# xuanvinh1997/llm-fp8

Hardware: AMD Instinct MI355X
Metric: train tokens/sec + FP8 GEMM % of MFMA peak, Llama-3.2-3B seq512 b16 (higher is better)
Workload: dtype fp8 (E4M3/E5M2 operands, fp32 accumulate, bf16 activations); 1 GPU; llama-3.2-3b (28 layers) full fine-tuning step, batch 16/GPU x seq 512, fp8_scenario=default (te_llama counterpart, lm_head FP8 under the outer recipe), random-init weights, synthetic tokens; route=fused, global_batch=16, seq_len=512, parallelism=single

## Files before the change

include/mi_fp8.h:

```cpp
#ifndef MI_FP8_H
#define MI_FP8_H

#include <stdint.h>

#ifdef __cplusplus
extern "C" {
#endif

#define MI_FMT_E4M3 0
#define MI_FMT_E5M2 1

#define MI_OK 0
#define MI_ERR_ARG (-1)
#define MI_ERR_SHAPE (-2)
#define MI_ERR_HIP (-3)

#define MI_OUT_BF16 0
#define MI_OUT_F32 1

#define MI_AMAX_ALGO_MAX 0
#define MI_AMAX_ALGO_MOST_RECENT 1

#define MI_ABI_VERSION 5
int mi_abi_version(void);
// ... 97 lines not shown
                        void* yT_fp8, const float* scale, float* amax, int64_t rows, int64_t cols, int fmt, void* stream);

int mi_sumsq_bf16(const void* g_bf16, int64_t n, float* partial, int n_partials, void* stream);
int mi_sumsq_bf16_multi(const int64_t* table, int n_tensors, const int32_t* chunks, int n_chunks, int chunk_elems,
                        double* partial, void* stream);
int mi_adamw_bf16_multi(const int64_t* table, int n_tensors, const int32_t* chunks, int n_chunks, int chunk_elems,
                        const float* grad_scale, float lr, float beta1, float beta2, float eps, float weight_decay,
                        int64_t step, void* stream);
int mi_adamw_cast_bf16_multi(const int64_t* table, int n_tensors, const int32_t* chunks, int n_chunks, int chunk_elems,
                             const float* grad_scale, float lr, float beta1, float beta2, float eps, float weight_decay,
                             int64_t step, void* stream);
int mi_adamw_mxcast_bf16_multi(const int64_t* table, int n_tensors, const int32_t* chunks, int n_chunks, int chunk_elems,
                               const float* grad_scale, float lr, float beta1, float beta2, float eps, float weight_decay,
                               int64_t step, void* stream);

int mi_embedding_grad_add(void* grad_bf16, const void* dy_bf16, const int64_t* sorted_ids, const int64_t* perm, int64_t tokens,
                          int64_t hidden, int64_t vocab, float alpha, int64_t padding_idx, void* stream);
int mi_adamw_bf16(void* p_bf16, const void* g_bf16, void* exp_avg_bf16, void* exp_avg_sq_bf16, int64_t n,
                  const float* grad_scale, float lr, float beta1, float beta2, float eps, float weight_decay,
                  int64_t step, void* stream);

int mi_attn_fwd(const void* q, const void* k, const void* v, void* o, float* lse, int B, int S, int H, int G, int D,
                int64_t q_ts, int64_t k_ts, int64_t v_ts, int64_t o_ts, float scale, int causal, void* stream);
#ifdef MI_DIAG
int mi_attn_fwd_diag(const void* q, const void* k, const void* v, void* o, float* lse, unsigned long long* dbg, int B, int S,
                     int H, int G, int D, int64_t q_ts, int64_t k_ts, int64_t v_ts, int64_t o_ts, float scale, void* stream);
#endif
int mi_attn_bwd(const void* q, const void* k, const void* v, const void* o, const void* dout, const float* lse,
                float* delta, void* dq, void* dk, void* dv, int B, int S, int H, int G, int D, int64_t q_ts,
                int64_t k_ts, int64_t v_ts, int64_t o_ts, int64_t do_ts, int64_t dq_ts, int64_t dk_ts, int64_t dv_ts,
                float scale, int causal, void* stream);

#ifdef __cplusplus
}
#endif
#endif
```

llm_fp8_amd/_lib.py:

```python
from __future__ import annotations

import ctypes
import os

_HERE = os.path.dirname(os.path.abspath(__file__))
LIB_PATH = os.environ.get("LLM_FP8_AMD_LIB") or os.path.join(_HERE, "libmi_fp8.so")
LAB_LIB_PATH = os.path.join(os.path.dirname(_HERE), "tools", "bin", "libmi_fp8_lab.so")

MI_FMT_E4M3 = 0
MI_FMT_E5M2 = 1
ABI_VERSION = 5

_c_i64 = ctypes.c_int64
_c_int = ctypes.c_int
_p = ctypes.c_void_p

class GemmProblem(ctypes.Structure):
    _fields_ = [("A", ctypes.c_void_p), ("B", ctypes.c_void_p), ("D", ctypes.c_void_p), ("sa_inv", ctypes.c_void_p),
                ("sb_inv", ctypes.c_void_p), ("M", ctypes.c_int64), ("N", ctypes.c_int64), ("K", ctypes.c_int64),
                ("lda", ctypes.c_int64), ("ldb", ctypes.c_int64), ("ldd", ctypes.c_int64)]


class GemmMxProblem(ctypes.Structure):
    _fields_ = [("A", ctypes.c_void_p), ("SA", ctypes.c_void_p), ("B", ctypes.c_void_p), ("SB", ctypes.c_void_p),
# ... 22 lines not shown
    "mi_rmsnorm_bwd": [_p, _p, _p, _p, _p, _p, _p, _c_int, _c_i64, _c_i64, _p],
    "mi_ce_forward": [_p, _p, _p, _p, _c_i64, _c_i64, _p],
    "mi_ce_backward": [_p, _p, _p, _p, _p, _c_i64, _c_i64, _p],
    "mi_ce_backward_cast": [_p, _p, _p, _p, _p, _p, _p, _p, _c_i64, _c_i64, _c_int, _p],
    "mi_sumsq_bf16": [_p, _c_i64, _p, _c_int, _p],
    "mi_sumsq_bf16_multi": [_p, _c_int, _p, _c_int, _c_int, _p, _p],
    "mi_adamw_bf16_multi": [_p, _c_int, _p, _c_int, _c_int, _p, ctypes.c_float, ctypes.c_float, ctypes.c_float, ctypes.c_float,
                            ctypes.c_float, _c_i64, _p],
    "mi_adamw_cast_bf16_multi": [_p, _c_int, _p, _c_int, _c_int, _p, ctypes.c_float, ctypes.c_float, ctypes.c_float, ctypes.c_float,
                                 ctypes.c_float, _c_i64, _p],
    "mi_adamw_mxcast_bf16_multi": [_p, _c_int, _p, _c_int, _c_int, _p, ctypes.c_float, ctypes.c_float, ctypes.c_float, ctypes.c_float,
                                   ctypes.c_float, _c_i64, _p],
    "mi_embedding_grad_add": [_p, _p, _p, _p, _c_i64, _c_i64, _c_i64, ctypes.c_float, _c_i64, _p],
    "mi_adamw_bf16": [_p, _p, _p, _p, _c_i64, _p, ctypes.c_float, ctypes.c_float, ctypes.c_float, ctypes.c_float,
                      ctypes.c_float, _c_i64, _p],
    "mi_add_rmsnorm_stats": [_p, _p, _p, _p, _c_i64, _c_i64, ctypes.c_float, _p],
    "mi_cast_amax_colsum": [_p, _p, _p, _p, _p, _p, _c_i64, _c_i64, _c_i64, _c_i64, _c_int, _p],
    "mi_colsum_finish": [_p, _c_i64, _c_i64, _p, _c_int, _p],
    "mi_colsum_finish_multi": [_p, _p, _p, _p, _p, _c_int, _p],
    "mi_gemm_workspace_bytes": [],
    "mi_gemm_set_workspace": [_p, _c_i64],
    "mi_attn_fwd": [_p, _p, _p, _p, _p, _c_int, _c_int, _c_int, _c_int, _c_int, _c_i64, _c_i64, _c_i64, _c_i64, ctypes.c_float,
                    _c_int, _p],
    "mi_attn_bwd": [_p] * 10 + [_c_int] * 5 + [_c_i64] * 8 + [ctypes.c_float, _c_int, _p],
    "mi_mxfp8_norm_quantize": [_p, _p, _p, _p, _p, _p, _p, _c_i64, _c_i64, _c_int, _p],
    "mi_mxfp8_swiglu_quantize": [_p, _p, _p, _p, _p, _c_i64, _c_i64, _c_int, _p],
    "mi_mxfp8_dswiglu_quantize": [_p, _p, _p, _p, _p, _p, _p, _c_i64, _c_i64, _c_int, _p],
    "mi_gemm_mxfp8": [_p, _p, _p, _p, _p, _p, _c_i64, _c_i64, _c_i64, _c_int, _c_int, _c_int, _c_int, _p],
    "mi_swiglu_cast_bias": [_p, _p, _p, _p, _p, _p, _c_i64, _c_i64, _c_int, _p],
    "mi_dswiglu_cast_bias": [_p, _p, _p, _p, _p, _p, _p, _p, _c_i64, _c_i64, _c_int, _p],
    "mi_add_bias_rmsnorm_stats": [_p, _p, _p, _p, _p, _c_i64, _c_i64, ctypes.c_float, _p],
    "mi_gemm_fp8_clock": [_p, _p, _p, _p, _p, _c_i64, _c_i64, _c_i64, _c_i64, _c_i64, _c_i64, _c_int, _p, _p],
}
LAB_SIGNATURES = {
    "mi_attn_fwd_diag": [_p, _p, _p, _p, _p, _p, _c_int, _c_int, _c_int, _c_int, _c_int, _c_i64, _c_i64, _c_i64, _c_i64, ctypes.c_float, _p],
}

_lib = None


def _bind(path: str, signatures) -> ctypes.CDLL:
    lib = ctypes.CDLL(path)
    for name, argtypes in signatures.items():
        fn = getattr(lib, name)
        fn.argtypes = argtypes
        fn.restype = ctypes.c_char_p if name == "mi_last_error" else (_c_i64 if name == "mi_gemm_workspace_bytes" else _c_int)
# ... 37 lines not shown
```

llm_fp8_amd/csrc/mi_attn.hip:

```cpp
#include "mi_common.h"

namespace mi {

typedef __bf16 bf8 __attribute__((ext_vector_type(8)));
typedef short s4v __attribute__((ext_vector_type(4)));
typedef short s8v __attribute__((ext_vector_type(8)));
typedef float f16v __attribute__((ext_vector_type(16)));
typedef __attribute__((address_space(3))) s4v lds_s4v;

template <int D>
__device__ __forceinline__ int tile_off(int row, int ch) {
  if (D == 128) return 256 * row + 16 * (ch ^ (((row & 3) << 2) | ((row >> 2) & 3)));
  return 128 * row + 16 * (ch ^ (((row & 1) << 2) | ((row >> 1) & 3)));
}

__device__ __forceinline__ bf8 as_bf8(v4i v) { return __builtin_bit_cast(bf8, v); }

template <int D>
__device__ __forceinline__ bf8 row_frag(const char* tile, int r0, int t, int lane) {
  const int r = lane & 31, h = lane >> 5;
  return as_bf8(*reinterpret_cast<const v4i*>(tile + tile_off<D>(r0 + r, 2 * t + h)));
}

template <int D>
// ... 28 lines not shown
constexpr int ATT_KB = 64;

typedef __amdgpu_buffer_rsrc_t rsrc_t;
#define MI_LDS_PTR(p) ((__attribute__((address_space(3))) void*)(p))
template <int D>
__device__ __forceinline__ void dma_voffsets(int* voff, int64_t tok_stride, int tid) {
  const int lane = tid & 63, w = tid >> 6;
#pragma unroll
  for (int i = 0; i < D / 32; ++i) {
    const int p = (4 * i + w) * 1024 + 16 * lane;
    const int row = p / (2 * D), slot = (p % (2 * D)) / 16;
    const int ch = D == 128 ? slot ^ (((row & 3) << 2) | ((row >> 2) & 3)) : slot ^ (((row & 1) << 2) | ((row >> 1) & 3));
    voff[i] = (int)((int64_t)row * tok_stride * 2) + 16 * ch;
  }
}
template <int D>
__device__ __forceinline__ void stage_dma(rsrc_t rs, const int* voff, int soff, char* tile, int w) {
#pragma unroll
  for (int i = 0; i < D / 32; ++i)
    __builtin_amdgcn_raw_ptr_buffer_load_lds(rs, MI_LDS_PTR(tile + (4 * i + w) * 1024), 16, voff[i], soff, 0, 0);
}
__device__ __forceinline__ void dma_wait_all() { asm volatile("s_waitcnt vmcnt(0)" ::: "memory"); }

template <int D, bool CAUSAL, bool DIAG = false>
__global__ __launch_bounds__(256, 2) void attn_fwd_kernel(const uint16_t* __restrict__ q, const uint16_t* __restrict__ k,
                                                          const uint16_t* __restrict__ v, uint16_t* __restrict__ o,
                                                          float* __restrict__ lse, int S, int H, int G, int64_t q_ts,
                                                          int64_t k_ts, int64_t v_ts, int64_t o_ts, float c,
                                                          unsigned long long* __restrict__ dbg = nullptr) {
  constexpr int TILE = ATT_KB * D * 2;
  constexpr int KT = D / 16, DB = D / 32;
  __shared__ __attribute__((aligned(16))) char lds[4 * TILE];
  const int tid = threadIdx.x, lane = tid & 63, w = tid >> 6, r = lane & 31, h = lane >> 5;
  const int qb = gridDim.x - 1 - blockIdx.x, head = blockIdx.y, b = blockIdx.z, g = head / (H / G);
  const int q_first = qb * ATT_QB + w * 32;
  const int qrow = q_first + r;
  const int ntiles = CAUSAL ? (qb * ATT_QB + ATT_QB) / ATT_KB : S / ATT_KB;
  const uint16_t* kbase = k + (int64_t)b * S * k_ts + (int64_t)g * D;
  const uint16_t* vbase = v + (int64_t)b * S * v_ts + (int64_t)g * D;

  bf8 qf[KT];
  {
    const uint16_t* qp = q + ((int64_t)b * S + qrow) * q_ts + (int64_t)head * D + 8 * h;
#pragma unroll
    for (int t = 0; t < KT; ++t) qf[t] = as_bf8(*reinterpret_cast<const v4i*>(qp + 16 * t));
  }
#pragma unroll
  for (int t = 0; t < KT; ++t) retire(qf[t]);
  f16v oacc[DB];
#pragma unroll
  for (int d = 0; d < DB; ++d)
#pragma unroll
// ... 119 lines not shown

  l += __shfl_xor(l, 32);
  const float inv = 1.0f / l;
  if (h == 0) lse[((int64_t)b * H + head) * S + qrow] = m * c + __builtin_amdgcn_logf(l);
  char* ot = lds + w * (32 * D * 2);
#pragma unroll
  for (int d = 0; d < DB; ++d)
#pragma unroll
    for (int i = 0; i < 4; ++i) {
      const int ch = 4 * d + i;
      uint2 pk;
      pk.x = pack_bf16x2(oacc[d][4 * i] * inv, oacc[d][4 * i + 1] * inv);
      pk.y = pack_bf16x2(oacc[d][4 * i + 2] * inv, oacc[d][4 * i + 3] * inv);
      *reinterpret_cast<uint2*>(ot + r * (D * 2) + 16 * (ch ^ (r & (D / 8 - 1))) + 8 * h) = pk;
    }
  __builtin_amdgcn_s_waitcnt(0xc07f);
  __builtin_amdgcn_wave_barrier();
  constexpr int CPR = D / 8;
#pragma unroll
  for (int it = 0; it < 32 * CPR / 64; ++it) {
    const int idx = it * 64 + lane, row = idx / CPR, ch = idx % CPR;
    const v4i val = *reinterpret_cast<const v4i*>(ot + row * (D * 2) + 16 * (ch ^ (row & (CPR - 1))));
    *reinterpret_cast<v4i*>(o + ((int64_t)b * S + q_first + row) * o_ts + (int64_t)head * D + ch * 8) = val;
  }
}


template <int D>
__device__ __forceinline__ void store_rows_from_accT(const f16v (&acc)[D / 32], float mul, char* slice, uint16_t* out,
                                                     int64_t row_stride, int lane) {
  const int r = lane & 31, h = lane >> 5;
  constexpr int CPR = D / 8;
#pragma unroll
  for (int d = 0; d < D / 32; ++d)
#pragma unroll
    for (int i = 0; i < 4; ++i) {
      const int ch = 4 * d + i;
      uint2 pk;
      pk.x = pack_bf16x2(acc[d][4 * i] * mul, acc[d][4 * i + 1] * mul);
      pk.y = pack_bf16x2(acc[d][4 * i + 2] * mul, acc[d][4 * i + 3] * mul);
      *reinterpret_cast<uint2*>(slice + r * (D * 2) + 16 * (ch ^ (r & (CPR - 1))) + 8 * h) = pk;
    }
  __builtin_amdgcn_s_waitcnt(0xc07f);
  __builtin_amdgcn_wave_barrier();
#pragma unroll
  for (int it = 0; it < 32 * CPR / 64; ++it) {
// ... 240 lines not shown
        const bf8 pf = acc_frag(sacc, s), dsf = acc_frag(dsacc, s);
#pragma unroll
        for (int d = 0; d < DB; ++d) {
          dva[d] = __builtin_amdgcn_mfma_f32_32x32x16_bf16(tr_frag<D>(dt, 16 * s, 32 * d, lane), pf, dva[d], 0, 0, 0);
          dka[d] = __builtin_amdgcn_mfma_f32_32x32x16_bf16(tr_frag<D>(qt, 16 * s, 32 * d, lane), dsf, dka[d], 0, 0, 0);
        }
      }
    }
    if (D == 128) {
#pragma unroll
      for (int d = 0; d < DB; ++d) asm volatile("" : "+a"(dka[d]), "+a"(dva[d]));
    }
    if (more) store_step(lds + ((step + 1) & 1) * BUF);
    __syncthreads();
  }
  char* slice = lds + w * SL;
  store_rows_from_accT<D>(dka, scale, slice, dk + ((int64_t)b * S + key_first) * dk_ts + (int64_t)g * D, dk_ts, lane);
  __builtin_amdgcn_wave_barrier();
  store_rows_from_accT<D>(dva, 1.0f, slice, dv + ((int64_t)b * S + key_first) * dv_ts + (int64_t)g * D, dv_ts, lane);
}

}

extern "C" int mi_attn_fwd(const void* q, const void* k, const void* v, void* o, float* lse, int B, int S, int H, int G,
                           int D, int64_t q_ts, int64_t k_ts, int64_t v_ts, int64_t o_ts, float scale, int causal,
                           void* stream) {
  MI_CHECK_ARG(q && k && v && o && lse, "mi_attn_fwd: null pointer");
  MI_CHECK_ARG(B >= 1 && H >= 1 && G >= 1 && H % G == 0, "mi_attn_fwd: bad B/H/G (%d, %d, %d)", B, H, G);
  MI_CHECK_ARG(D == 128 || D == 64, "mi_attn_fwd: head_dim %d not supported (64, 128)", D);
  MI_CHECK_ARG(S >= 128 && S % 128 == 0, "mi_attn_fwd: seq %d must be a multiple of 128", S);
  MI_CHECK_ARG(q_ts % 8 == 0 && k_ts % 8 == 0 && v_ts % 8 == 0 && o_ts % 8 == 0, "mi_attn_fwd: token strides must be multiples of 8");
  MI_CHECK_ARG((int64_t)S * k_ts * 2 < (1LL << 31) && (int64_t)S * v_ts * 2 < (1LL << 31) && ((uintptr_t)k % 16) == 0 && ((uintptr_t)v % 16) == 0,
               "mi_attn_fwd: one batch of K / V must span < 2 GiB and be 16-byte aligned (32-bit buffer offsets of the LDS DMA)");
  MI_CHECK_ARG(((uintptr_t)q % 16) == 0 && ((uintptr_t)o % 16) == 0, "mi_attn_fwd: q and o must be 16-byte aligned (16-byte row accesses)");
  MI_CHECK_ARG(H <= 65535 && B <= 65535, "mi_attn_fwd: grid too large");
  const float c = scale * 1.4426950408889634f;
  dim3 grid(S / mi::ATT_QB, H, B), block(256);
  hipStream_t st = (hipStream_t)stream;
#define MI_ATTN_FWD(DD, CC)                                                                                            \
  hipLaunchKernelGGL((mi::attn_fwd_kernel<DD, CC>), grid, block, 0, st, (const uint16_t*)q, (const uint16_t*)k,          \
                     (const uint16_t*)v, (uint16_t*)o, lse, S, H, G, q_ts, k_ts, v_ts, o_ts, c, (unsigned long long*)nullptr)
  if (D == 128) {
    if (causal) MI_ATTN_FWD(128, true); else MI_ATTN_FWD(128, false);
  } else {
    if (causal) MI_ATTN_FWD(64, true); else MI_ATTN_FWD(64, false);
  }
#undef MI_ATTN_FWD
  MI_CHECK_LAUNCH("mi_attn_fwd launch");
  return MI_OK;
}

#ifdef MI_DIAG
extern "C" int mi_attn_fwd_diag(const void* q, const void* k, const void* v, void* o, float* lse, unsigned long long* dbg, int B,
                                int S, int H, int G, int D, int64_t q_ts, int64_t k_ts, int64_t v_ts, int64_t o_ts, float scale,
                                void* stream) {
  MI_CHECK_ARG(q && k && v && o && lse && dbg, "mi_attn_fwd_diag: null pointer");
  MI_CHECK_ARG(D == 128 && S % 128 == 0 && H % G == 0, "mi_attn_fwd_diag: unsupported shape");
  dim3 grid(S / mi::ATT_QB, H, B), block(256);
  hipLaunchKernelGGL((mi::attn_fwd_kernel<128, true, true>), grid, block, 0, (hipStream_t)stream, (const uint16_t*)q,
                     (const uint16_t*)k, (const uint16_t*)v, (uint16_t*)o, lse, S, H, G, q_ts, k_ts, v_ts, o_ts,
                     scale * 1.4426950408889634f, dbg);
  MI_CHECK_LAUNCH("mi_attn_fwd_diag launch");
  return MI_OK;
}
#endif

extern "C" int mi_attn_bwd(const void* q, const void* k, const void* v, const void* o, const void* dout, const float* lse,
                           float* delta, void* dq, void* dk, void* dv, int B, int S, int H, int G, int D, int64_t q_ts,
                           int64_t k_ts, int64_t v_ts, int64_t o_ts, int64_t do_ts, int64_t dq_ts, int64_t dk_ts,
                           int64_t dv_ts, float scale, int causal, void* stream) {
  MI_CHECK_ARG(q && k && v && o && dout && lse && delta && dq && dk && dv, "mi_attn_bwd: null pointer");
  MI_CHECK_ARG(B >= 1 && H >= 1 && G >= 1 && H % G == 0, "mi_attn_bwd: bad B/H/G (%d, %d, %d)", B, H, G);
// ... 30 lines not shown
```

llm_fp8_amd/pytorch/attention.py:

```python
from __future__ import annotations

import os
import weakref
from typing import Optional

import torch
import torch.nn.functional as F

from . import ops
from .module import DyHandoff, LayerNormLinear, Linear, handoff_readers

__all__ = ["RotaryPositionEmbedding", "apply_rotary_pos_emb", "DotProductAttention", "MultiheadAttention"]


class RotaryPositionEmbedding(torch.nn.Module):

    def __init__(self, dim: int, rotary_percent: float = 1.0, seq_len_interpolation_factor=None,
                 pretrained_max_position_embeddings=None, rotary_base: float = 10000.0):
        super().__init__()
        if rotary_percent < 1.0:
            dim = int(dim * rotary_percent)
        self.dim = dim
        self.seq_len_interpolation_factor = seq_len_interpolation_factor
        inv_freq = 1.0 / (rotary_base ** (torch.arange(0, dim, 2, dtype=torch.float32) / dim))
# ... 60 lines not shown
        cos, sin = ctx.saved_tensors
        B, S, n_q, n_kv, d = ctx.meta
        T = B * S
        h = ctx.handoff
        if h is not None and h.offered() and handoff_readers(ctx.act_ref()):
            h = None
        if h is not None and h.offered() and d == 128 and T % (32 if h.mx else 8) == 0:
            args = (dq.reshape(T, n_q * d), dk.reshape(T, n_kv * d), dv.reshape(T, n_kv * d), cos, sin, n_q, n_kv, d, S)
            if h.mx:
                fp8 = ops.mxfp8_rope_bwd_quantize(*args, h.fmt, rowwise=h.want_y, colwise=h.want_t)
            else:
                fp8 = ops.rope_qkv_backward_cast(*args, h.scale, h.amax, h.fmt, want_y=h.want_y, want_t=h.want_t)
            g = torch.empty((B, S, (n_q + 2 * n_kv) * d), dtype=torch.bfloat16, device=dq.device)
            h.put(fp8, g)
            return g, None, None, None, None, None, None
        g = ops.rope_qkv_backward(dq.reshape(T, n_q * d), dk.reshape(T, n_kv * d), dv.reshape(T, n_kv * d), cos, sin,
                                  n_q, n_kv, d, S)
        return g.view(B, S, -1), None, None, None, None, None, None


class _FlashAttnFn(torch.autograd.Function):

    @staticmethod
    def forward(ctx, q, k, v, scale, causal):
        o, lse = ops.attn_fwd(q, k, v, scale, causal)
        ctx.save_for_backward(q, k, v, o, lse)
        ctx.scale, ctx.causal = scale, causal
        return o

    @staticmethod
    def backward(ctx, do):
        q, k, v, o, lse = ctx.saved_tensors
        ok = (do.stride(3) == 1 and do.stride(2) == do.shape[3] and do.stride(0) == do.shape[1] * do.stride(1)
              and do.stride(1) % 8 == 0 and do.data_ptr() % 16 == 0)
        do = do if ok else do.clone(memory_format=torch.contiguous_format)
        dq, dk, dv = ops.attn_bwd(do, q, k, v, o, lse, ctx.scale, ctx.causal)
        return dq, dk, dv, None, None


def _flash_ok(q, k, v, causal: bool, dropout: float) -> bool:
    if not (q.is_cuda and q.dtype == k.dtype == v.dtype == torch.bfloat16 and dropout == 0.0 and causal):
        return False
    B, S, H, D = q.shape
    if D not in (64, 128) or S % 128 or S < 128 or H % k.shape[2]:
        return False
    return all(t.stride(3) == 1 and t.stride(2) == D and t.stride(0) == S * t.stride(1) and t.stride(1) % 8 == 0
               and S * t.stride(1) * 2 < 2 ** 31 and t.data_ptr() % 16 == 0 for t in (q, k, v))


class DotProductAttention(torch.nn.Module):

    def __init__(self, num_attention_heads: int, kv_channels: int, num_gqa_groups: Optional[int] = None,
                 attention_dropout: float = 0.0, attn_mask_type: str = "causal", qkv_format: str = "bshd", **_ignored):
        super().__init__()
        self.h, self.d = num_attention_heads, kv_channels
        self.g = num_gqa_groups or num_attention_heads
        self.p, self.attn_mask_type, self.qkv_format = attention_dropout, attn_mask_type, qkv_format

    def forward(self, q, k, v, attention_mask=None):
        if self.qkv_format == "sbhd":
            q, k, v = (t.transpose(0, 1) for t in (q, k, v))
        causal = self.attn_mask_type in ("causal", "padding_causal")
        if _flash_ok(q, k, v, causal, self.p if self.training else 0.0):
            o = _FlashAttnFn.apply(q, k, v, self.d ** -0.5, True)
            if self.qkv_format == "sbhd":
                o = o.transpose(0, 1)
            return o.reshape(*o.shape[:2], self.h * self.d)
        q, k, v = (t.transpose(1, 2) for t in (q, k, v))
        mask = None
        if not causal and attention_mask is not None:
            mask = ~attention_mask if attention_mask.dtype == torch.bool else attention_mask
        o = F.scaled_dot_product_attention(q, k, v, attn_mask=mask, dropout_p=self.p if self.training else 0.0,
                                           is_causal=causal, enable_gqa=(self.g != self.h))
        o = o.transpose(1, 2)
        if self.qkv_format == "sbhd":
            o = o.transpose(0, 1)
        return o.reshape(*o.shape[:2], self.h * self.d)


class MultiheadAttention(torch.nn.Module):

    def __init__(self, hidden_size: int, num_attention_heads: int, kv_channels: Optional[int] = None,
                 attention_dropout: float = 0.1, layernorm_epsilon: float = 1e-5, init_method=None,
                 output_layer_init_method=None, attn_mask_type: str = "causal", num_gqa_groups: Optional[int] = None,
                 input_layernorm: bool = False, attention_type: str = "self", fuse_qkv_params: bool = False,
                 zero_centered_gamma: bool = False, qkv_weight_interleaved: bool = True, bias: bool = True,
                 normalization: str = "LayerNorm", qkv_format: str = "sbhd", params_dtype=None, device="cuda",
# ... 21 lines not shown
                              init_method=init_method)
        self.core_attention = DotProductAttention(self.h, self.d, self.g, attention_dropout, attn_mask_type, qkv_format)
        self.proj = Linear(q_out, hidden_size, bias=bias, params_dtype=params_dtype, device=device,
                           init_method=output_layer_init_method or init_method)

    def forward(self, hidden_states: torch.Tensor, attention_mask: Optional[torch.Tensor] = None,
                rotary_pos_emb=None, _with_skip: bool = False, _rstd=None, **_ignored):
        if _with_skip:
            if not self.input_layernorm:
                return self._attend(self.qkv(hidden_states), attention_mask, rotary_pos_emb), hidden_states
            handoff = DyHandoff() if (rotary_pos_emb is not None and hidden_states.is_cuda and torch.is_grad_enabled()
                                      and os.environ.get("LLM_FP8_AMD_NO_DY_HANDOFF") != "1") else None
            qkv, skip = self.layernorm_qkv(hidden_states, _with_skip=True, _rstd=_rstd, _dy_handoff=handoff)
            return self._attend(qkv, attention_mask, rotary_pos_emb, handoff), skip
        qkv = self.layernorm_qkv(hidden_states) if self.input_layernorm else self.qkv(hidden_states)
        return self._attend(qkv, attention_mask, rotary_pos_emb)

    def _attend(self, qkv: torch.Tensor, attention_mask, rotary_pos_emb, handoff=None) -> torch.Tensor:
        if (rotary_pos_emb is not None and not isinstance(rotary_pos_emb, (tuple, list)) and qkv.is_cuda
                and qkv.dtype == torch.bfloat16 and self.qkv_format == "bshd" and self.d % 16 == 0
                and rotary_pos_emb.shape[-1] == self.d):
            cos, sin = _cos_sin_tables(rotary_pos_emb, qkv.shape[1])
            q, k, v = _RoPESplitFn.apply(qkv, cos, sin, self.h, self.g, self.d, handoff)
            return self.proj(self.core_attention(q, k, v, attention_mask))
        if handoff is not None:
            handoff.withdraw()
        q, k, v = torch.split(qkv, self.split, dim=-1)
        a, b = qkv.shape[0], qkv.shape[1]
        q = q.reshape(a, b, self.h, self.d)
        k = k.reshape(a, b, self.g, self.d)
        v = v.reshape(a, b, self.g, self.d)
        if rotary_pos_emb is not None:
            fq, fk = rotary_pos_emb if isinstance(rotary_pos_emb, (tuple, list)) else (rotary_pos_emb, rotary_pos_emb)
            q = apply_rotary_pos_emb(q, fq, self.qkv_format)
            k = apply_rotary_pos_emb(k, fk, self.qkv_format)
        ctx = self.core_attention(q, k, v, attention_mask)
        return self.proj(ctx)
```

llm_fp8_amd/pytorch/module.py:

```python
from __future__ import annotations

import io
import os
from typing import List, Optional, Sequence, Tuple

import torch
import torch.nn.functional as F

from ..common.recipe import DelayedScaling, Format, MXFP8BlockScaling, Recipe, fmt_codes
from . import ops
from .fp8 import FP8GlobalStateManager, ModuleMeta

__all__ = ["Linear", "LayerNormLinear", "LayerNormMLP", "LayerNorm", "RMSNorm"]


def _as_bf16_2d(t: torch.Tensor) -> torch.Tensor:
    t2 = t.reshape(-1, t.shape[-1])
    if t2.dtype != torch.bfloat16:
        t2 = t2.to(torch.bfloat16)
    return t2.contiguous()


class DyHandoff:
    __slots__ = ("scale", "amax", "fmt", "want_y", "want_t", "fp8", "ptr", "mx", "act_ref")
# ... 3 lines not shown
        self.act_ref = None
        self.want_y = self.want_t = self.mx = False

    def offer(self, scale, amax, fmt, want_y, want_t, mx: bool = False):
        self.scale, self.amax, self.fmt, self.want_y, self.want_t, self.mx = scale, amax, fmt, want_y, want_t, mx

    def withdraw(self):
        self.scale, self.mx = None, False

    def offered(self) -> bool:
        return (self.scale is not None or self.mx) and (self.want_y or self.want_t)

    def put(self, fp8: tuple, placeholder: torch.Tensor):
        self.fp8, self.ptr = fp8, placeholder.untyped_storage().data_ptr()

    def take(self, dy: torch.Tensor):
        if dy.untyped_storage().data_ptr() != self.ptr:
            raise RuntimeError("DyHandoff: the gradient reaching the Linear is not the producer's placeholder "
                               "(an op was inserted between the q|k|v projection and the rotary split)")
        fp8, self.fp8, self.ptr = self.fp8, None, None
        return fp8


def handoff_readers(t) -> bool:
    if torch.is_anomaly_enabled():
        return True
    if t is None:
        return False
    return bool(getattr(t, "retains_grad", False)) or bool(getattr(t, "_backward_hooks", None))


class _GemmSpec:
    __slots__ = ("recipe", "meta_fwd", "meta_bwd", "g", "fmt_fwd", "fmt_bwd", "trigger_bwd_update", "training", "eps",
                 "wcache", "first_mb", "with_skip", "rstd", "dy_handoff", "defer_bias", "q")

    def __init__(self, recipe, meta_fwd, meta_bwd, g, trigger_bwd_update, training, eps=1e-5, wcache=None, first_mb=None,
                 with_skip=False, rstd=None, dy_handoff=None, defer_bias=False):
        self.dy_handoff = dy_handoff
        self.defer_bias = defer_bias
        self.eps = eps
        self.rstd = rstd
        self.with_skip = with_skip
        self.wcache, self.first_mb = wcache, first_mb
        self.recipe, self.meta_fwd, self.meta_bwd, self.g = recipe, meta_fwd, meta_bwd, g
        self.fmt_fwd, self.fmt_bwd = fmt_codes(recipe.fp8_format)
        self.q = _MXQ(self.fmt_fwd, self.fmt_bwd) if recipe.mxfp8() else _DelayedQ(meta_fwd, meta_bwd, self.fmt_fwd, self.fmt_bwd)
        self.trigger_bwd_update = trigger_bwd_update
        self.training = training


class _Sink:
    __slots__ = ("parts", "stamp")

    def _register(self, weights, ns, attr: str) -> None:
        self.parts, r = [], 0
        for w, n in zip(weights, ns):
            self.parts.append((w, r, n))
            setattr(w, attr, (self, r, n))
            r += n
        self.stamp = None

# ... 77 lines not shown




class _DelayedQ:
    __slots__ = ("mf", "mb", "fmt_f", "fmt_b")
    mx = False
    cache_key, sink_key = "ds", "sink"
    no_sink = "row-sharded weights of this shape cannot take an FP8 sink"
    swiglu_adds_bias = True
    colsum_dtypes = None

    def __init__(self, mf, mb, fmt_f: int, fmt_b: int):
        self.mf, self.mb, self.fmt_f, self.fmt_b = mf, mb, fmt_f, fmt_b

    def _act(self, y, yT, s: int):
        return (y, self.mf.scale_inv(s)), (yT, self.mf.scale_inv_snapshot()[s:s + 1])

    def quantize(self, x2, g: int, want_t: bool, norm=None):
        mf, s = self.mf, 3 * g
        if norm is None:
            return self._act(*ops.cast_amax(x2, mf.scale(s), mf.amax(s), self.fmt_f, want_t=want_t), s)
        return self._act(*ops.norm_cast(x2, norm[0], norm[1], mf.scale(s), mf.amax(s), self.fmt_f, want_t=want_t), s)

    def swiglu(self, h, g: int, want_t: bool, bias):
        mf, s = self.mf, 3 * g
        return self._act(*ops.swiglu_cast(h, mf.scale(s), mf.amax(s), self.fmt_f, want_t=want_t, bias=bias), s)

    def _grad(self, y, yT, cs, s: int):
        si = self.mb.scale_inv(s)
        return (y, si), (yT, si), cs

    def quantize_grad(self, g2, g: int, want_y: bool, want_t: bool, colsum: bool = False):
        mb, s = self.mb, 2 * g
        out = ops.cast_amax(g2, mb.scale(s), mb.amax(s), self.fmt_b, want_y=want_y, want_t=want_t, want_colsum=colsum)
        return self._grad(out[0], out[1], out[2] if colsum else None, s)

    def dswiglu(self, h, dact, g: int, want_y: bool, want_t: bool, colsum: bool, bias):
        mb, s = self.mb, 2 * g
        return self._grad(*ops.dswiglu_cast(h, dact, mb.scale(s), mb.amax(s), self.fmt_b, want_y=want_y, want_t=want_t,
                                            want_colsum=colsum, bias=bias), s)

    def offer(self, handoff: DyHandoff, g: int, want_y: bool, want_t: bool) -> None:
        if self.mb is not None:
            handoff.offer(self.mb.scale(2 * g), self.mb.amax(2 * g), self.fmt_b, want_y, want_t)

# ... 200 lines not shown
            dx = torch.empty((M, K), dtype=torch.bfloat16, device=g8.device)
            dw = dw_out if dw_out is not None else torch.empty((N, K), dtype=torch.bfloat16, device=g8.device)
            probs = [dgrad + (dx,), wgrad + (dw,)]
            cfg = ops.grouped_gemm_choice(probs, fmt_b, fmt_f, mx=mx)
            if cfg >= 0:
                (ops.gemm_mxfp8_grouped if mx else ops.gemm_fp8_grouped)(probs, fmt_b, fmt_f, tile_cfg=cfg)
                return dx, dw
    gemm = ops.gemm_mxfp8 if mx else ops.gemm_fp8
    dx = gemm(*dgrad, fmt_b, fmt_f) if need_dgrad else None
    dw = gemm(*wgrad, fmt_b, fmt_f, out=dw_out) if need_wgrad else None
    return dx, dw


def _skip_2d(dskip: Optional[torch.Tensor], like: torch.Tensor) -> Optional[torch.Tensor]:
    if dskip is None:
        return None
    d = dskip.reshape(like.shape)
    return d if (d.dtype == torch.bfloat16 and d.is_contiguous()) else d.to(torch.bfloat16).contiguous()


def _quantize_input(ctx, spec: _GemmSpec, x2, ln_w, want_t: bool, need_dgrad: bool):
    ctx.norm = None
    if ln_w is None:
        return spec.q.quantize(x2, spec.g, want_t)
    gam = (ln_w if ln_w.dtype == torch.bfloat16 else ln_w.to(torch.bfloat16)).contiguous()
    rstd = spec.rstd if spec.rstd is not None else ops.rmsnorm_stats(x2, spec.eps)
    if need_dgrad:
        ctx.norm = (x2, rstd, gam, ln_w.dtype)
    return spec.q.quantize(x2, spec.g, want_t, (rstd, gam))


def _finish_dx(ctx, dx, dskip, colsums=None):
    dln = None
    if ctx.norm is not None and dx is not None:
        xin, rstd, gam, ln_dtype = ctx.norm
        ctx.norm = None
        dx, dln = ops.rmsnorm_bwd(dx, xin, rstd, gam, dres=_skip_2d(dskip, dx), dgamma_dtype=ln_dtype, finish=colsums is None)
        dskip = None
        if colsums is not None:
            dln = (dln, ln_dtype)
    if colsums is not None:
        pend = [t for t in (*colsums, dln) if t is not None]
        if pend:
            done = iter(ops.colsum_finish_multi(pend))
            colsums = [None if t is None else next(done) for t in colsums]
            dln = None if dln is None else next(done)
# ... 215 lines not shown
        return _layernorm(x, self.weight, self.bias, self.eps, self.zero_centered_gamma)


def _init_weight(shape, dtype, device, init_method=None):
    w = torch.empty(shape, dtype=dtype, device=device)
    if init_method is not None:
        init_method(w)
    else:
        torch.nn.init.normal_(w, mean=0.0, std=0.023)
    return torch.nn.Parameter(w)


class Linear(_FP8Module):

    def __init__(self, in_features: int, out_features: int, bias: bool = True, params_dtype=None, device="cuda",
                 init_method=None, **_ignored):
        super().__init__()
        self.in_features, self.out_features = in_features, out_features
        dt = params_dtype or torch.get_default_dtype()
        self.weight = _init_weight((out_features, in_features), dt, device, init_method)
        self.bias = torch.nn.Parameter(torch.zeros(out_features, dtype=dt, device=device)) if bias else None
        self.use_bias = bias

    def forward(self, inp: torch.Tensor, is_first_microbatch=None) -> torch.Tensor:
        st = self._prepare(inp.device)
        if st is None:
            if getattr(self, "_pending_norm", None) is not None:
                raise RuntimeError("Linear: a deferred RMSNorm is pending but FP8 is off for this forward")
            return F.linear(inp, _master(self.weight).to(inp.dtype), None if self.bias is None else self.bias.to(inp.dtype))
        handoff = DyHandoff() if (getattr(self, "offer_dy_handoff", False) and self.training and torch.is_grad_enabled()
                                  and self.bias is None) else None
        pn, self._pending_norm = getattr(self, "_pending_norm", None), None
        ln_w, eps, rstd = None, 1e-5, None
        if pn is not None:
            ln_w, eps, rs, ptr, shape = pn
            if inp.data_ptr() != ptr or tuple(inp.shape) != shape:
                raise RuntimeError("Linear: a deferred RMSNorm is pending for another tensor than the one this forward received")
            rstd = _usable_rstd(rs, inp, eps)
        y = _FP8LinearFn.apply(inp, self.bias, self._spec(st, is_first_microbatch, eps=eps, rstd=rstd, dy_handoff=handoff), ln_w,
                               self.weight)
        if handoff is not None and handoff.offered():
            y._mi_dy_handoff = handoff
        return y

    def extra_repr(self):
        return f"in_features={self.in_features}, out_features={self.out_features}, bias={self.use_bias}"


class LayerNormLinear(_FP8Module):

    def __init__(self, in_features: int, out_features: int, eps: float = 1e-5, bias: bool = True,
                 normalization: str = "LayerNorm", parameters_split=None, params_dtype=None, device="cuda",
                 zero_centered_gamma: bool = False, init_method=None, return_layernorm_output: bool = False, **_ignored):
        super().__init__()
        assert normalization in ("LayerNorm", "RMSNorm")
        self.in_features, self.out_features, self.eps = in_features, out_features, eps
        self.normalization, self.zero_centered_gamma = normalization, zero_centered_gamma
        self.return_layernorm_output = return_layernorm_output
        dt = params_dtype or torch.get_default_dtype()
        self.layer_norm_weight = torch.nn.Parameter(
            torch.zeros(in_features, dtype=dt, device=device) if zero_centered_gamma else torch.ones(in_features, dtype=dt, device=device))
        self.layer_norm_bias = (torch.nn.Parameter(torch.zeros(in_features, dtype=dt, device=device))
                                if normalization == "LayerNorm" else None)
# ... 130 lines not shown
```

llm_fp8_amd/pytorch/ops.py:

```python
from __future__ import annotations

import ctypes
import os
from typing import Optional, Tuple

import torch

from .. import _lib
from .profiler import KernelTimer

E4M3, E5M2 = _lib.MI_FMT_E4M3, _lib.MI_FMT_E5M2
FP8_MAX = {E4M3: 448.0, E5M2: 57344.0}


_SK_WORKSPACE = {}


def ensure_gemm_workspace(device: torch.device) -> None:
    idx = device.index if device.index is not None else torch.cuda.current_device()
    if idx in _SK_WORKSPACE:
        return
    lib = _lib.load()
    with torch.cuda.device(idx):
        nbytes = int(lib.mi_gemm_workspace_bytes())
# ... 672 lines not shown
    for t in (q, k, v):
        _bshd_ok(t, D)
    if out is None:
        o = torch.empty((B, S, H, D), dtype=torch.bfloat16, device=q.device)
        lse = torch.empty((B, H, S), dtype=torch.float32, device=q.device)
    else:
        o, lse = out
        _dev(o, lse)
        _bshd_ok(o, D)
        assert o.shape == q.shape and lse.shape == (B, H, S) and lse.dtype == torch.float32 and lse.is_contiguous()
    args = (q.data_ptr(), k.data_ptr(), v.data_ptr(), o.data_ptr(), lse.data_ptr(), B, S, H, G, D, q.stride(1), k.stride(1),
            v.stride(1), o.stride(1), float(scale), int(causal), _stream())
    t = KernelTimer.active
    flops = 4.0 * B * H * S * S * D * (0.5 if causal else 1.0)
    if t is None:
        rc = _lib.load().mi_attn_fwd(*args)
    else:
        with t.span("attn_fwd", f"{B}x{S}x{H}x{D}", flops, 2.0 * (q.numel() * 2 + k.numel() * 2)):
            rc = _lib.load().mi_attn_fwd(*args)
    _lib.check(rc, "mi_attn_fwd")
    return o, lse


def attn_bwd(do: torch.Tensor, q: torch.Tensor, k: torch.Tensor, v: torch.Tensor, o: torch.Tensor, lse: torch.Tensor,
             scale: float, causal: bool = True, out=None):
    _dev(do, q, k, v, o, lse)
    B, S, H, D = q.shape
    G = k.shape[2]
    for t in (q, k, v, o, do):
        _bshd_ok(t, D)
    assert o.shape == do.shape == q.shape and lse.shape == (B, H, S) and lse.dtype == torch.float32 and lse.is_contiguous()
    if out is None:
        dq = torch.empty((B, S, H, D), dtype=torch.bfloat16, device=q.device)
        dk = torch.empty((B, S, G, D), dtype=torch.bfloat16, device=q.device)
        dv = torch.empty((B, S, G, D), dtype=torch.bfloat16, device=q.device)
    else:
        dq, dk, dv = out
        _dev(dq, dk, dv)
        for t in out:
            _bshd_ok(t, D)
        assert dq.shape == q.shape and dk.shape == dv.shape == k.shape
    delta = torch.empty((B, H, S), dtype=torch.float32, device=q.device)
    args = (q.data_ptr(), k.data_ptr(), v.data_ptr(), o.data_ptr(), do.data_ptr(), lse.data_ptr(), delta.data_ptr(),
            dq.data_ptr(), dk.data_ptr(), dv.data_ptr(), B, S, H, G, D, q.stride(1), k.stride(1), v.stride(1), o.stride(1),
            do.stride(1), dq.stride(1), dk.stride(1), dv.stride(1), float(scale), int(causal), _stream())
    t = KernelTimer.active
# ... 9 lines not shown
```

Before: 88980 tokens/s.

## Fuse FP8 cast and transpose of attention output into flash-attention forward

```diff
diff --git a/include/mi_fp8.h b/include/mi_fp8.h
--- a/include/mi_fp8.h
+++ b/include/mi_fp8.h
@@ -143,6 +143,9 @@
 
 int mi_attn_fwd(const void* q, const void* k, const void* v, void* o, float* lse, int B, int S, int H, int G, int D,
                 int64_t q_ts, int64_t k_ts, int64_t v_ts, int64_t o_ts, float scale, int causal, void* stream);
+int mi_attn_fwd_cast(const void* q, const void* k, const void* v, void* o, float* lse, void* o8, void* o8T,
+                     const float* o8_scale, float* o8_amax, int B, int S, int H, int G, int D, int64_t q_ts, int64_t k_ts,
+                     int64_t v_ts, int64_t o_ts, int64_t ld8, int64_t ld8T, int fmt, float scale, int causal, void* stream);
 #ifdef MI_DIAG
 int mi_attn_fwd_diag(const void* q, const void* k, const void* v, void* o, float* lse, unsigned long long* dbg, int B, int S,
                      int H, int G, int D, int64_t q_ts, int64_t k_ts, int64_t v_ts, int64_t o_ts, float scale, void* stream);
diff --git a/llm_fp8_amd/_lib.py b/llm_fp8_amd/_lib.py
--- a/llm_fp8_amd/_lib.py
+++ b/llm_fp8_amd/_lib.py
@@ -68,6 +68,7 @@
     "mi_gemm_set_workspace": [_p, _c_i64],
     "mi_attn_fwd": [_p, _p, _p, _p, _p, _c_int, _c_int, _c_int, _c_int, _c_int, _c_i64, _c_i64, _c_i64, _c_i64, ctypes.c_float,
                     _c_int, _p],
+    "mi_attn_fwd_cast": [_p] * 9 + [_c_int] * 5 + [_c_i64] * 6 + [_c_int, ctypes.c_float, _c_int, _p],
     "mi_attn_bwd": [_p] * 10 + [_c_int] * 5 + [_c_i64] * 8 + [ctypes.c_float, _c_int, _p],
     "mi_mxfp8_norm_quantize": [_p, _p, _p, _p, _p, _p, _p, _c_i64, _c_i64, _c_int, _p],
     "mi_mxfp8_swiglu_quantize": [_p, _p, _p, _p, _p, _c_i64, _c_i64, _c_int, _p],
diff --git a/llm_fp8_amd/csrc/mi_attn.hip b/llm_fp8_amd/csrc/mi_attn.hip
--- a/llm_fp8_amd/csrc/mi_attn.hip
+++ b/llm_fp8_amd/csrc/mi_attn.hip
@@ -74,12 +74,15 @@
 }
 __device__ __forceinline__ void dma_wait_all() { asm volatile("s_waitcnt vmcnt(0)" ::: "memory"); }
 
-template <int D, bool CAUSAL, bool DIAG = false>
+template <int D, bool CAUSAL, bool DIAG = false, int EMIT = -1>
 __global__ __launch_bounds__(256, 2) void attn_fwd_kernel(const uint16_t* __restrict__ q, const uint16_t* __restrict__ k,
                                                           const uint16_t* __restrict__ v, uint16_t* __restrict__ o,
                                                           float* __restrict__ lse, int S, int H, int G, int64_t q_ts,
                                                           int64_t k_ts, int64_t v_ts, int64_t o_ts, float c,
-                                                          unsigned long long* __restrict__ dbg = nullptr) {
+                                                          unsigned long long* __restrict__ dbg = nullptr,
+                                                          uint8_t* __restrict__ o8 = nullptr, uint8_t* __restrict__ o8T = nullptr,
+                                                          const float* __restrict__ scale_p = nullptr, float* amax_out = nullptr,
+                                                          int64_t ld8 = 0, int64_t ld8T = 0) {
   constexpr int TILE = ATT_KB * D * 2;
   constexpr int KT = D / 16, DB = D / 32;
   __shared__ __attribute__((aligned(16))) char lds[4 * TILE];
@@ -245,6 +248,83 @@
     const int idx = it * 64 + lane, row = idx / CPR, ch = idx % CPR;
     const v4i val = *reinterpret_cast<const v4i*>(ot + row * (D * 2) + 16 * (ch ^ (row & (CPR - 1))));
     *reinterpret_cast<v4i*>(o + ((int64_t)b * S + q_first + row) * o_ts + (int64_t)head * D + ch * 8) = val;
+  }
+  if constexpr (EMIT >= 0) {
+    constexpr int CB = D / 8;
+    char* tt = lds + 4 * (32 * D * 2);
+    float* s_amax = reinterpret_cast<float*>(tt + D * 128);
+    const bool act = lane < 4 * CB;
+    const int rb = lane / CB, cb = lane % CB;
+    const float qscale = *scale_p;
+    float amax = 0.0f;
+    if (act) {
+      v4i raw[8];
+#pragma unroll
+      for (int i = 0; i < 8; ++i) {
+        const int row = 8 * rb + i;
+        raw[i] = *reinterpret_cast<const v4i*>(ot + row * (D * 2) + 16 * (cb ^ (row & (CPR - 1))));
+      }
+      u32 screen = 0;
+#pragma unroll
+      for (int i = 0; i < 8; ++i)
+#pragma unroll
+        for (int j = 0; j < 4; ++j) screen = nan_screen(screen, (u32)raw[i][j]);
+      const bool has_nan = nan_seen(screen);
+      u32 lo[8], hi[8];
+#pragma unroll
+      for (int i = 0; i < 8; ++i) {
+        float f[8];
+#pragma unroll
+        for (int j = 0; j < 4; ++j) {
+          u32 wd = (u32)raw[i][j];
+          f[2 * j] = __uint_as_float(wd << 16);
+          f[2 * j + 1] = __uint_as_float(wd & 0xFFFF0000u);
+        }
+        if (__builtin_expect(has_nan, 0)) {
+#pragma unroll
+          for (int j = 0; j < 8; ++j) amax = fmaxf(amax, (f[j] != f[j]) ? 0.0f : fabsf(f[j]));
+        } else {
+#pragma unroll
+          for (int j = 0; j < 8; ++j) amax = fmaxf(amax, fabsf(f[j]));
+        }
+        lo[i] = cvt4_fp8<EMIT>(f[0] * qscale, f[1] * qscale, f[2] * qscale, f[3] * qscale);
+        hi[i] = cvt4_fp8<EMIT>(f[4] * qscale, f[5] * qscale, f[6] * qscale, f[7] * qscale);
+      }
+      uint8_t* dst = o8 + ((int64_t)b * S + q_first + 8 * rb) * ld8 + (int64_t)head * D + 8 * cb;
+#pragma unroll
+      for (int i = 0; i < 8; ++i) mi::st8<MI_NT_Y>(dst + (int64_t)i * ld8, lo[i], hi[i]);
+      if (o8T != nullptr) {
+        u32 ta[4], tb[4], tc[4], td[4];
+        transpose4x4(lo[0], lo[1], lo[2], lo[3], ta[0], ta[1], ta[2], ta[3]);
+        transpose4x4(lo[4], lo[5], lo[6], lo[7], tb[0], tb[1], tb[2], tb[3]);
+        transpose4x4(hi[0], hi[1], hi[2], hi[3], tc[0], tc[1], tc[2], tc[3]);
+        transpose4x4(hi[4], hi[5], hi[6], hi[7], td[0], td[1], td[2], td[3]);
+        const int gr = 4 * w + rb;
+        char* col = tt + (8 * cb) * 128 + 16 * ((gr >> 1) ^ (cb & 7)) + 8 * (gr & 1);
+#pragma unroll
+        for (int j = 0; j < 4; ++j) {
+          *reinterpret_cast<uint2*>(col + j * 128) = make_uint2(ta[j], tb[j]);
+          *reinterpret_cast<uint2*>(col + (j + 4) * 128) = make_uint2(tc[j], td[j]);
+        }
+      }
+    }
+    amax = wave_max(amax);
+    if (lane == 0) s_amax[w] = amax;
+    __syncthreads();
+    if (o8T != nullptr) {
+      uint8_t* dstT = o8T + (int64_t)head * D * ld8T + (int64_t)b * S + (int64_t)qb * ATT_QB;
+#pragma unroll
+      for (int it = 0; it < D / 32; ++it) {
+        const int idx = it * 256 + tid, cc = idx >> 3, ch = idx & 7;
+        const v4i val = *reinterpret_cast<const v4i*>(tt + cc * 128 + 16 * (ch ^ ((cc >> 3) & 7)));
+        if (MI_NT_YT) __builtin_nontemporal_store(val, reinterpret_cast<v4i*>(dstT + (int64_t)cc * ld8T + 16 * ch));
+        else *reinterpret_cast<v4i*>(dstT + (int64_t)cc * ld8T + 16 * ch) = val;
+      }
+    }
+    if (amax_out != nullptr && tid == 0) {
+      const float mm = fmaxf(fmaxf(s_amax[0], s_amax[1]), fmaxf(s_amax[2], s_amax[3]));
+      if (mm > 0.0f && mm > __builtin_nontemporal_load(amax_out)) atomicMax(reinterpret_cast<unsigned int*>(amax_out), __float_as_uint(mm));
+    }
   }
 }
 
@@ -531,32 +611,64 @@
 
 }
 
+static int attn_fwd_impl(const char* who, const void* q, const void* k, const void* v, void* o, float* lse, void* o8, void* o8T,
+                         const float* o8_scale, float* o8_amax, int B, int S, int H, int G, int D, int64_t q_ts, int64_t k_ts,
+                         int64_t v_ts, int64_t o_ts, int64_t ld8, int64_t ld8T, int fmt, float scale, int causal, void* stream) {
+  MI_CHECK_ARG(q && k && v && o && lse, "%s: null pointer", who);
+  MI_CHECK_ARG(B >= 1 && H >= 1 && G >= 1 && H % G == 0, "%s: bad B/H/G (%d, %d, %d)", who, B, H, G);
+  MI_CHECK_ARG(D == 128 || D == 64, "%s: head_dim %d not supported (64, 128)", who, D);
+  MI_CHECK_ARG(S >= 128 && S % 128 == 0, "%s: seq %d must be a multiple of 128", who, S);
+  MI_CHECK_ARG(q_ts % 8 == 0 && k_ts % 8 == 0 && v_ts % 8 == 0 && o_ts % 8 == 0, "%s: token strides must be multiples of 8", who);
+  MI_CHECK_ARG((int64_t)S * k_ts * 2 < (1LL << 31) && (int64_t)S * v_ts * 2 < (1LL << 31) && ((uintptr_t)k % 16) == 0 && ((uintptr_t)v % 16) == 0,
+               "%s: one batch of K / V must span < 2 GiB and be 16-byte aligned (32-bit buffer offsets of the LDS DMA)", who);
+  MI_CHECK_ARG(((uintptr_t)q % 16) == 0 && ((uintptr_t)o % 16) == 0, "%s: q and o must be 16-byte aligned (16-byte row accesses)", who);
+  MI_CHECK_ARG(H <= 65535 && B <= 65535, "%s: grid too large", who);
+  if (fmt >= 0) {
+    MI_CHECK_ARG(fmt == MI_FMT_E4M3 || fmt == MI_FMT_E5M2, "%s: bad fmt %d", who, fmt);
+    MI_CHECK_ARG(o8 && o8_scale, "%s: o8 and its scale must be non-null", who);
+    MI_CHECK_ARG(ld8 >= (int64_t)H * D && ld8 % 8 == 0 && ((uintptr_t)o8 % 8) == 0,
+                 "%s: ld8 must be >= H * D and a multiple of 8, o8 8-byte aligned", who);
+    MI_CHECK_ARG(!o8T || (ld8T >= (int64_t)B * S && ld8T % 16 == 0 && ((uintptr_t)o8T % 16) == 0),
+                 "%s: ld8T must be >= B * S and a multiple of 16, o8T 16-byte aligned", who);
+  }
+  const float c = scale * 1.4426950408889634f;
+  dim3 grid(S / mi::ATT_QB, H, B), block(256);
+  hipStream_t st = (hipStream_t)stream;
+#define MI_ATTN_FWD(DD, CC, EE)                                                                                        \
+  hipLaunchKernelGGL((mi::attn_fwd_kernel<DD, CC, false, EE>), grid, block, 0, st, (const uint16_t*)q, (const uint16_t*)k, \
+                     (const uint16_t*)v, (uint16_t*)o, lse, S, H, G, q_ts, k_ts, v_ts, o_ts, c, (unsigned long long*)nullptr, \
+                     (uint8_t*)o8, (uint8_t*)o8T, o8_scale, o8_amax, ld8, ld8T)
+#define MI_ATTN_FWD_E(DD, CC)                                   \
+  do {                                                          \
+    if (fmt < 0) MI_ATTN_FWD(DD, CC, -1);                       \
+    else if (fmt == MI_FMT_E4M3) MI_ATTN_FWD(DD, CC, MI_FMT_E4M3); \
+    else MI_ATTN_FWD(DD, CC, MI_FMT_E5M2);                      \
+  } while (0)
+  if (D == 128) {
+    if (causal) MI_ATTN_FWD_E(128, true); else MI_ATTN_FWD_E(128, false);
+  } else {
+    if (causal) MI_ATTN_FWD_E(64, true); else MI_ATTN_FWD_E(64, false);
+  }
+#undef MI_ATTN_FWD_E
+#undef MI_ATTN_FWD
+  MI_CHECK_LAUNCH(who);
+  return MI_OK;
+}
+
 extern "C" int mi_attn_fwd(const void* q, const void* k, const void* v, void* o, float* lse, int B, int S, int H, int G,
                            int D, int64_t q_ts, int64_t k_ts, int64_t v_ts, int64_t o_ts, float scale, int causal,
                            void* stream) {
-  MI_CHECK_ARG(q && k && v && o && lse, "mi_attn_fwd: null pointer");
-  MI_CHECK_ARG(B >= 1 && H >= 1 && G >= 1 && H % G == 0, "mi_attn_fwd: bad B/H/G (%d, %d, %d)", B, H, G);
-  MI_CHECK_ARG(D == 128 || D == 64, "mi_attn_fwd: head_dim %d not supported (64, 128)", D);
-  MI_CHECK_ARG(S >= 128 && S % 128 == 0, "mi_attn_fwd: seq %d must be a multiple of 128", S);
-  MI_CHECK_ARG(q_ts % 8 == 0 && k_ts % 8 == 0 && v_ts % 8 == 0 && o_ts % 8 == 0, "mi_attn_fwd: token strides must be multiples of 8");
-  MI_CHECK_ARG((int64_t)S * k_ts * 2 < (1LL << 31) && (int64_t)S * v_ts * 2 < (1LL << 31) && ((uintptr_t)k % 16) == 0 && ((uintptr_t)v % 16) == 0,
-               "mi_attn_fwd: one batch of K / V must span < 2 GiB and be 16-byte aligned (32-bit buffer offsets of the LDS DMA)");
-  MI_CHECK_ARG(((uintptr_t)q % 16) == 0 && ((uintptr_t)o % 16) == 0, "mi_attn_fwd: q and o must be 16-byte aligned (16-byte row accesses)");
-  MI_CHECK_ARG(H <= 65535 && B <= 65535, "mi_attn_fwd: grid too large");
-  const float c = scale * 1.4426950408889634f;
-  dim3 grid(S / mi::ATT_QB, H, B), block(256);
-  hipStream_t st = (hipStream_t)stream;
-#define MI_ATTN_FWD(DD, CC)                                                                                            \
-  hipLaunchKernelGGL((mi::attn_fwd_kernel<DD, CC>), grid, block, 0, st, (const uint16_t*)q, (const uint16_t*)k,          \
-                     (const uint16_t*)v, (uint16_t*)o, lse, S, H, G, q_ts, k_ts, v_ts, o_ts, c, (unsigned long long*)nullptr)
-  if (D == 128) {
-    if (causal) MI_ATTN_FWD(128, true); else MI_ATTN_FWD(128, false);
-  } else {
-    if (causal) MI_ATTN_FWD(64, true); else MI_ATTN_FWD(64, false);
-  }
-#undef MI_ATTN_FWD
-  MI_CHECK_LAUNCH("mi_attn_fwd launch");
-  return MI_OK;
+  return attn_fwd_impl("mi_attn_fwd", q, k, v, o, lse, nullptr, nullptr, nullptr, nullptr, B, S, H, G, D, q_ts, k_ts, v_ts, o_ts,
+                       0, 0, -1, scale, causal, stream);
+}
+
+extern "C" int mi_attn_fwd_cast(const void* q, const void* k, const void* v, void* o, float* lse, void* o8, void* o8T,
+                                const float* o8_scale, float* o8_amax, int B, int S, int H, int G, int D, int64_t q_ts,
+                                int64_t k_ts, int64_t v_ts, int64_t o_ts, int64_t ld8, int64_t ld8T, int fmt, float scale,
+                                int causal, void* stream) {
+  MI_CHECK_ARG(fmt >= 0, "mi_attn_fwd_cast: bad fmt %d", fmt);
+  return attn_fwd_impl("mi_attn_fwd_cast", q, k, v, o, lse, o8, o8T, o8_scale, o8_amax, B, S, H, G, D, q_ts, k_ts, v_ts, o_ts,
+                       ld8, ld8T, fmt, scale, causal, stream);
 }
 
 #ifdef MI_DIAG
diff --git a/llm_fp8_amd/pytorch/attention.py b/llm_fp8_amd/pytorch/attention.py
--- a/llm_fp8_amd/pytorch/attention.py
+++ b/llm_fp8_amd/pytorch/attention.py
@@ -106,8 +106,13 @@
 class _FlashAttnFn(torch.autograd.Function):
 
     @staticmethod
-    def forward(ctx, q, k, v, scale, causal):
-        o, lse = ops.attn_fwd(q, k, v, scale, causal)
+    def forward(ctx, q, k, v, scale, causal, x_handoff=None):
+        if x_handoff is not None:
+            o, lse, o8, o8t = ops.attn_fwd_cast(q, k, v, scale, x_handoff.scale, x_handoff.amax, x_handoff.fmt, causal,
+                                                want_t=x_handoff.want_t)
+            x_handoff.put(o8, o8t, o)
+        else:
+            o, lse = ops.attn_fwd(q, k, v, scale, causal)
         ctx.save_for_backward(q, k, v, o, lse)
         ctx.scale, ctx.causal = scale, causal
         return o
@@ -119,7 +124,7 @@
               and do.stride(1) % 8 == 0 and do.data_ptr() % 16 == 0)
         do = do if ok else do.clone(memory_format=torch.contiguous_format)
         dq, dk, dv = ops.attn_bwd(do, q, k, v, o, lse, ctx.scale, ctx.causal)
-        return dq, dk, dv, None, None
+        return dq, dk, dv, None, None, None
 
 
 def _flash_ok(q, k, v, causal: bool, dropout: float) -> bool:
@@ -141,12 +146,12 @@
         self.g = num_gqa_groups or num_attention_heads
         self.p, self.attn_mask_type, self.qkv_format = attention_dropout, attn_mask_type, qkv_format
 
-    def forward(self, q, k, v, attention_mask=None):
+    def forward(self, q, k, v, attention_mask=None, _x_handoff=None):
         if self.qkv_format == "sbhd":
             q, k, v = (t.transpose(0, 1) for t in (q, k, v))
         causal = self.attn_mask_type in ("causal", "padding_causal")
         if _flash_ok(q, k, v, causal, self.p if self.training else 0.0):
-            o = _FlashAttnFn.apply(q, k, v, self.d ** -0.5, True)
+            o = _FlashAttnFn.apply(q, k, v, self.d ** -0.5, True, _x_handoff if self.qkv_format == "bshd" else None)
             if self.qkv_format == "sbhd":
                 o = o.transpose(0, 1)
             return o.reshape(*o.shape[:2], self.h * self.d)
@@ -214,7 +219,8 @@
                 and rotary_pos_emb.shape[-1] == self.d):
             cos, sin = _cos_sin_tables(rotary_pos_emb, qkv.shape[1])
             q, k, v = _RoPESplitFn.apply(qkv, cos, sin, self.h, self.g, self.d, handoff)
-            return self.proj(self.core_attention(q, k, v, attention_mask))
+            xh = self.proj.offer_input(q)
+            return self.proj(self.core_attention(q, k, v, attention_mask, _x_handoff=xh), _x_handoff=xh)
         if handoff is not None:
             handoff.withdraw()
         q, k, v = torch.split(qkv, self.split, dim=-1)
diff --git a/llm_fp8_amd/pytorch/module.py b/llm_fp8_amd/pytorch/module.py
--- a/llm_fp8_amd/pytorch/module.py
+++ b/llm_fp8_amd/pytorch/module.py
@@ -49,6 +49,28 @@
         return fp8
 
 
+class XHandoff:
+    __slots__ = ("st", "scale", "amax", "fmt", "want_t", "fp8", "key")
+
+    def __init__(self, st, scale, amax, fmt: int, want_t: bool):
+        self.st, self.scale, self.amax, self.fmt, self.want_t = st, scale, amax, fmt, want_t
+        self.fp8 = self.key = None
+
+    @staticmethod
+    def _key(x2: torch.Tensor):
+        return x2.data_ptr(), tuple(x2.shape), x2._version
+
+    def put(self, y: torch.Tensor, yT: Optional[torch.Tensor], x: torch.Tensor):
+        self.fp8, self.key = (y, yT), (x.data_ptr(), tuple(y.shape), x._version)
+
+    def take(self, x2: torch.Tensor, want_t: bool):
+        fp8, key = self.fp8, self.key
+        self.fp8 = self.key = None
+        if fp8 is None or key != self._key(x2) or not x2.is_contiguous() or (want_t and fp8[1] is None):
+            return None
+        return fp8
+
+
 def handoff_readers(t) -> bool:
     if torch.is_anomaly_enabled():
         return True
@@ -59,11 +81,12 @@
 
 class _GemmSpec:
     __slots__ = ("recipe", "meta_fwd", "meta_bwd", "g", "fmt_fwd", "fmt_bwd", "trigger_bwd_update", "training", "eps",
-                 "wcache", "first_mb", "with_skip", "rstd", "dy_handoff", "defer_bias", "q")
+                 "wcache", "first_mb", "with_skip", "rstd", "dy_handoff", "defer_bias", "q", "x_handoff")
 
     def __init__(self, recipe, meta_fwd, meta_bwd, g, trigger_bwd_update, training, eps=1e-5, wcache=None, first_mb=None,
-                 with_skip=False, rstd=None, dy_handoff=None, defer_bias=False):
+                 with_skip=False, rstd=None, dy_handoff=None, defer_bias=False, x_handoff=None):
         self.dy_handoff = dy_handoff
+        self.x_handoff = x_handoff
         self.defer_bias = defer_bias
         self.eps = eps
         self.rstd = rstd
@@ -187,6 +210,9 @@
         if norm is None:
             return self._act(*ops.cast_amax(x2, mf.scale(s), mf.amax(s), self.fmt_f, want_t=want_t), s)
         return self._act(*ops.norm_cast(x2, norm[0], norm[1], mf.scale(s), mf.amax(s), self.fmt_f, want_t=want_t), s)
+
+    def taken_input(self, fp8, g: int, want_t: bool):
+        return self._act(fp8[0], fp8[1] if want_t else None, 3 * g)
 
     def swiglu(self, h, g: int, want_t: bool, bias):
         mf, s = self.mf, 3 * g
@@ -433,6 +459,9 @@
 def _quantize_input(ctx, spec: _GemmSpec, x2, ln_w, want_t: bool, need_dgrad: bool):
     ctx.norm = None
     if ln_w is None:
+        got = spec.x_handoff.take(x2, want_t) if spec.x_handoff is not None else None
+        if got is not None:
+            return spec.q.taken_input(got, spec.g, want_t)
         return spec.q.quantize(x2, spec.g, want_t)
     gam = (ln_w if ln_w.dtype == torch.bfloat16 else ln_w.to(torch.bfloat16)).contiguous()
     rstd = spec.rstd if spec.rstd is not None else ops.rmsnorm_stats(x2, spec.eps)
@@ -694,8 +723,16 @@
         self.bias = torch.nn.Parameter(torch.zeros(out_features, dtype=dt, device=device)) if bias else None
         self.use_bias = bias
 
-    def forward(self, inp: torch.Tensor, is_first_microbatch=None) -> torch.Tensor:
-        st = self._prepare(inp.device)
+    def offer_input(self, like: torch.Tensor) -> Optional[XHandoff]:
+        if (os.environ.get("LLM_FP8_AMD_NO_X_HANDOFF") == "1" or not like.is_cuda or getattr(self, "_pending_norm", None) is not None
+                or not FP8GlobalStateManager.is_fp8_enabled() or not FP8GlobalStateManager.get_fp8_recipe().delayed()):
+            return None
+        st = self._prepare(like.device)
+        mf = st[1]
+        return XHandoff(st, mf.scale(0), mf.amax(0), fmt_codes(st[0].fp8_format)[0], torch.is_grad_enabled() and self.weight.requires_grad)
+
+    def forward(self, inp: torch.Tensor, is_first_microbatch=None, _x_handoff: Optional[XHandoff] = None) -> torch.Tensor:
+        st = self._prepare(inp.device) if _x_handoff is None else _x_handoff.st
         if st is None:
             if getattr(self, "_pending_norm", None) is not None:
                 raise RuntimeError("Linear: a deferred RMSNorm is pending but FP8 is off for this forward")
@@ -709,8 +746,8 @@
             if inp.data_ptr() != ptr or tuple(inp.shape) != shape:
                 raise RuntimeError("Linear: a deferred RMSNorm is pending for another tensor than the one this forward received")
             rstd = _usable_rstd(rs, inp, eps)
-        y = _FP8LinearFn.apply(inp, self.bias, self._spec(st, is_first_microbatch, eps=eps, rstd=rstd, dy_handoff=handoff), ln_w,
-                               self.weight)
+        y = _FP8LinearFn.apply(inp, self.bias, self._spec(st, is_first_microbatch, eps=eps, rstd=rstd, dy_handoff=handoff,
+                                                          x_handoff=_x_handoff), ln_w, self.weight)
         if handoff is not None and handoff.offered():
             y._mi_dy_handoff = handoff
         return y
diff --git a/llm_fp8_amd/pytorch/ops.py b/llm_fp8_amd/pytorch/ops.py
--- a/llm_fp8_amd/pytorch/ops.py
+++ b/llm_fp8_amd/pytorch/ops.py
@@ -718,6 +718,32 @@
     return o, lse
 
 
+def attn_fwd_cast(q: torch.Tensor, k: torch.Tensor, v: torch.Tensor, scale: float, x_scale: torch.Tensor,
+                  x_amax: Optional[torch.Tensor], fmt: int, causal: bool = True, want_t: bool = True):
+    _dev(q, k, v, x_scale, x_amax)
+    B, S, H, D = q.shape
+    G = k.shape[2]
+    for t in (q, k, v):
+        _bshd_ok(t, D)
+    assert x_scale.dtype == torch.float32 and (x_amax is None or x_amax.dtype == torch.float32)
+    o = torch.empty((B, S, H, D), dtype=torch.bfloat16, device=q.device)
+    lse = torch.empty((B, H, S), dtype=torch.float32, device=q.device)
+    o8 = torch.empty((B * S, H * D), dtype=torch.uint8, device=q.device)
+    o8T = torch.empty((H * D, B * S), dtype=torch.uint8, device=q.device) if want_t else None
+    args = (q.data_ptr(), k.data_ptr(), v.data_ptr(), o.data_ptr(), lse.data_ptr(), o8.data_ptr(), _ptr(o8T), x_scale.data_ptr(),
+            _ptr(x_amax), B, S, H, G, D, q.stride(1), k.stride(1), v.stride(1), o.stride(1), H * D, B * S, fmt, float(scale),
+            int(causal), _stream())
+    t = KernelTimer.active
+    if t is None:
+        rc = _lib.load().mi_attn_fwd_cast(*args)
+    else:
+        flops = 4.0 * B * H * S * S * D * (0.5 if causal else 1.0)
+        with t.span("attn_fwd", f"{B}x{S}x{H}x{D}+cast", flops, 2.0 * (q.numel() * 2 + k.numel() * 2) + o.numel() * (1 + int(want_t))):
+            rc = _lib.load().mi_attn_fwd_cast(*args)
+    _lib.check(rc, "mi_attn_fwd_cast")
+    return o, lse, o8, o8T
+
+
 def attn_bwd(do: torch.Tensor, q: torch.Tensor, k: torch.Tensor, v: torch.Tensor, o: torch.Tensor, lse: torch.Tensor,
              scale: float, causal: bool = True, out=None):
     _dev(do, q, k, v, o, lse)
```

Measured after the change: 89740 tokens/s, median of 6. Within noise of the previous version (+0.9%).
